# eladhoffer/convNet.pytorch

Hardware: NVIDIA H100
Metric: ResNet-50 images/sec (training step, synthetic 224x224) (higher is better)
Workload: dtype bf16

## Files before the change

### convnet/pytorch_b200/csrc/conv3x3.cu

```cuda
#include "common.cuh"
#include "host.h"
#include <stdlib.h>

namespace b200 {

constexpr int kHMaxA = 6, kHMaxB = 8;
constexpr int kHMaxTaps = 16;

struct HaloParams {
  int N, H, W, C, Kout;
  int RT, Wp;
  int tiles_per_img, m_tiles, n_tiles, block_n, c_chunks;
  int sa, sb;
  uint32_t a_bytes, a_box_bytes, b_bytes;
  int act;
  int has_res;
  double* stats;
  const float* bias;
  int ntaps, pad;
  int row_bytes;
  int b_stationary;
  int diag;
  uint16_t a_off[kHMaxTaps];
  uint16_t b_tap[kHMaxTaps];
};

template <int NTAPS, int KSTEPS, int BN>
__global__ void __launch_bounds__(kThreads, 1)
conv_halo_kernel(const __grid_constant__ CUtensorMap tmX, const __grid_constant__ CUtensorMap tmB,
                 const __grid_constant__ CUtensorMap tmC, const __grid_constant__ CUtensorMap tmR,
                 const __grid_constant__ HaloParams p) {
  extern __shared__ uint8_t smem_raw[];
  __shared__ __align__(8) uint64_t a_full[kHMaxA], a_empty[kHMaxA], b_full[kHMaxB], b_empty[kHMaxB];
  __shared__ __align__(8) uint64_t res_bar, bstat_bar;

  const int warp = threadIdx.x >> 5, lane = threadIdx.x & 31;
  const uint32_t raw_addr = smem_u32(smem_raw);
  uint8_t* smem = smem_raw + (((raw_addr + 1023u) & ~1023u) - raw_addr);
  uint8_t* sA = smem;
  uint8_t* sB = sA + p.sa * p.a_bytes;
  const int b_slots = p.b_stationary ? p.c_chunks * p.ntaps : p.sb;
  uint8_t* epi = sB + b_slots * p.b_bytes;

  if (threadIdx.x == 0) {
    for (int i = 0; i < p.sa; ++i) { mbar_init(&a_full[i], 1); mbar_init(&a_empty[i], 8); }
    for (int i = 0; i < kHMaxB; ++i) { mbar_init(&b_full[i], 1); mbar_init(&b_empty[i], 8); }
    mbar_init(&bstat_bar, 1);
    mbar_init(&res_bar, 1);
    fence_mbar_init();
    prefetch_tmap(&tmX); prefetch_tmap(&tmB); prefetch_tmap(&tmC);
    if (p.has_res) prefetch_tmap(&tmR);
  }
  __syncthreads();
  const int t_start = p.diag ? static_cast<int>(blockIdx.x) / p.n_tiles : static_cast<int>(blockIdx.x);
  const int t_step = p.diag ? static_cast<int>(gridDim.x) / p.n_tiles : static_cast<int>(gridDim.x);
  const int total_tiles = p.diag ? p.m_tiles : p.m_tiles * p.n_tiles;
  const int own_n = static_cast<int>(blockIdx.x) % p.n_tiles;

  if (warp >= 8) {
    producer_setmaxnreg();
    if (warp == 8 && lane == 0) {
      int ia = 0, ib = 0; uint32_t pa = 0, pb = 0;
      const int cw = p.row_bytes >> 1;
      if (p.b_stationary && t_start < total_tiles) {
        mbar_arrive_expect_tx(&bstat_bar, static_cast<uint32_t>(p.c_chunks * NTAPS) * p.b_bytes);
        for (int cc = 0; cc < p.c_chunks; ++cc)
          for (int t = 0; t < NTAPS; ++t)
            tma_load_3d(&tmB, &bstat_bar, sB + (cc * NTAPS + t) * p.b_bytes, cc * cw, p.b_tap[t],
                        p.diag ? own_n * p.block_n : 0);
      }
      for (int tile = t_start; tile < total_tiles; tile += t_step) {
        const int m_tile = p.diag ? tile : tile / p.n_tiles, n_tile = p.diag ? own_n : tile - m_tile * p.n_tiles;
        const int img = m_tile / p.tiles_per_img;
        const int h0 = (m_tile - img * p.tiles_per_img) * p.RT;
        for (int cc = 0; cc < p.c_chunks; ++cc) {
          mbar_wait(&a_empty[ia], pa ^ 1u);
          mbar_arrive_expect_tx(&a_full[ia], p.a_box_bytes);
          tma_load_4d(&tmX, &a_full[ia], sA + ia * p.a_bytes, (p.diag ? n_tile : cc) * cw, -p.pad, h0 - p.pad, img);
          if (++ia == p.sa) { ia = 0; pa ^= 1u; }
          if (p.b_stationary) continue;
          for (int t = 0; t < NTAPS; ++t) {
            mbar_wait(&b_empty[ib], pb ^ 1u);
            mbar_arrive_expect_tx(&b_full[ib], p.b_bytes);
            tma_load_3d(&tmB, &b_full[ib], sB + ib * p.b_bytes, cc * cw, p.b_tap[t], n_tile * p.block_n);
            if (++ib == p.sb) { ib = 0; pb ^= 1u; }
          }
        }
      }
    }
    return;
  }
  consumer_setmaxnreg();

  const int wg = warp >> 2;
  const int r_lo = wg * 64 + (warp & 3) * 16 + (lane >> 2);
  const int c_lo = 2 * (lane & 3);
  const bool leader = threadIdx.x == 0;
  const uint64_t proto = make_smem_desc(0, 16, 8u * p.row_bytes, layout_type_for_row_bytes(p.row_bytes));
  const uint32_t a_wg = (64u * wg * p.row_bytes) >> 4;
  const int nbox = BN >> 6;
  const uint32_t box_bytes = static_cast<uint32_t>(p.RT * p.W) * 128u;
  const uint32_t box_pitch = (box_bytes + 1023u) & ~1023u;
  int srow[2];
  bool in_tile[2];
#pragma unroll
  for (int h = 0; h < 2; ++h) {
    const int v = r_lo + 8 * h;
    const int ry = v / p.Wp, cx = v - ry * p.Wp;
    srow[h] = ry * p.W + cx;
    in_tile[h] = (ry < p.RT) && (cx < p.W);
  }
  const int st_col = threadIdx.x % BN;
  const int st_rows = kTileM / (256 / BN);
  const int st_row0 = (threadIdx.x / BN) * st_rows;
  int st_ntile = -1;
  float st_s1 = 0.f, st_s2 = 0.f;
  if (p.b_stationary && t_start < total_tiles) mbar_wait(&bstat_bar, 0);

  float acc[BN / 2];
  int ia = 0, ib = 0; uint32_t pa = 0, pb = 0;
  int local = 0;
  for (int tile = t_start; tile < total_tiles; tile += t_step, ++local) {
    const int m_tile = p.diag ? tile : tile / p.n_tiles, n_tile = p.diag ? own_n : tile - m_tile * p.n_tiles;
    const int img = m_tile / p.tiles_per_img;
    const int h0 = (m_tile - img * p.tiles_per_img) * p.RT;
    const int nbase = n_tile * BN;
    if (leader && local > 0) bulk_wait_group_read0();
    named_bar_sync(1, 256);
    if (leader && p.has_res) {
      fence_proxy_async();
      mbar_arrive_expect_tx(&res_bar, static_cast<uint32_t>(nbox) * box_bytes);
      for (int b = 0; b < nbox; ++b) tma_load_4d(&tmR, &res_bar, epi + b * box_pitch, nbase + b * 64, 0, h0, img);
    }

    wgmma_fence_acc(acc);
    int rel_a = -1, rel_b = -1;
    for (int cc = 0; cc < p.c_chunks; ++cc) {
      mbar_wait(&a_full[ia], pa);
      const uint64_t da0 = proto + (smem_u32(sA + ia * p.a_bytes) >> 4) + a_wg;
#pragma unroll
      for (int t = 0; t < NTAPS; ++t) {
        uint64_t db0;
        if (p.b_stationary) {
          db0 = proto + (smem_u32(sB + (cc * NTAPS + t) * p.b_bytes) >> 4);
        } else {
          mbar_wait(&b_full[ib], pb);
          db0 = proto + (smem_u32(sB + ib * p.b_bytes) >> 4);
        }
        const uint32_t tap_inc = (static_cast<uint32_t>(p.a_off[t]) * p.row_bytes) >> 4;
        wgmma_fence();
#pragma unroll
        for (int k = 0; k < KSTEPS; ++k)
          wgmma_bf16<0, 0>(acc, da0 + tap_inc + 2 * k, db0 + 2 * k, (cc | t | k) != 0 ? 1u : 0u);
        if (!p.b_stationary || t == NTAPS - 1) {
          wgmma_commit();
          wgmma_wait<1>();
          if (rel_b >= 0) release_stage(&b_empty[rel_b], lane);
          if (rel_a >= 0) release_stage(&a_empty[rel_a], lane);
          rel_a = (t == NTAPS - 1) ? ia : -1;
          rel_b = p.b_stationary ? -1 : ib;
        }
        if (!p.b_stationary && ++ib == p.sb) { ib = 0; pb ^= 1u; }
      }
      if (++ia == p.sa) { ia = 0; pa ^= 1u; }
    }
    wgmma_wait<0>();
    wgmma_fence_acc(acc);
    if (rel_b >= 0) release_stage(&b_empty[rel_b], lane);
    if (rel_a >= 0) release_stage(&a_empty[rel_a], lane);

    if (p.has_res) mbar_wait(&res_bar, static_cast<uint32_t>(local & 1));
#pragma unroll
    for (int h = 0; h < 2; ++h) {
      if (!in_tile[h] || h0 + (r_lo + 8 * h) / p.Wp >= p.H) continue;
      const int row = srow[h];
#pragma unroll
      for (int j = 0; j < BN / 2; j += 4) {
        const int c = 2 * j + c_lo;
        uint32_t* dst = reinterpret_cast<uint32_t*>(epi + staged_offset(row, c, box_pitch));
        float v0 = acc[j + 2 * h], v1 = acc[j + 2 * h + 1];
        if (p.bias != nullptr) { v0 += __ldg(p.bias + nbase + c); v1 += __ldg(p.bias + nbase + c + 1); }
        if (p.has_res) {
          const float2 t2 = unpack_bf16x2(*dst);
          v0 += t2.x;
          v1 += t2.y;
        }
        *dst = pack_bf16x2(apply_act(v0, p.act), apply_act(v1, p.act));
      }
    }
    fence_proxy_async();
    named_bar_sync(1, 256);
    if (leader) {
      for (int b = 0; b < nbox; ++b) tma_store_4d(&tmC, epi + b * box_pitch, nbase + b * 64, 0, h0, img);
      bulk_commit_group();
    }
    if (p.stats != nullptr) {
      if (st_ntile != n_tile) {
        if (st_ntile >= 0) flush_bn_stats(p.stats, p.Kout, st_ntile * BN, st_col, st_s1, st_s2);
        st_ntile = n_tile; st_s1 = 0.f; st_s2 = 0.f;
      }
      const int vrows = min(p.RT, p.H - h0) * p.W;
      const int r_end = min(st_row0 + st_rows, vrows);
      for (int r = st_row0; r < r_end; ++r) {
        const float x = __bfloat162float(*reinterpret_cast<const __nv_bfloat16*>(epi + staged_offset(r, st_col, box_pitch)));
        st_s1 += x;
        st_s2 = fmaf(x, x, st_s2);
      }
    }
  }
  if (p.stats != nullptr && st_ntile >= 0) flush_bn_stats(p.stats, p.Kout, st_ntile * BN, st_col, st_s1, st_s2);
  if (leader) bulk_wait_group0();
}

typedef void (*HaloKernelFn)(const __grid_constant__ CUtensorMap, const __grid_constant__ CUtensorMap,
                             const __grid_constant__ CUtensorMap, const __grid_constant__ CUtensorMap,
                             const __grid_constant__ HaloParams);
static HaloKernelFn halo_kernel_for(int ntaps, int block_n) {
  if (ntaps == 9)
    return block_n == 64 ? conv_halo_kernel<9, 4, 64> : block_n == 128 ? conv_halo_kernel<9, 4, 128>
         : block_n == 256 ? conv_halo_kernel<9, 4, 256> : nullptr;
  if (ntaps == 16)
    return block_n == 64 ? conv_halo_kernel<16, 1, 64> : block_n == 128 ? conv_halo_kernel<16, 1, 128>
         : block_n == 256 ? conv_halo_kernel<16, 1, 256> : nullptr;
  return nullptr;
}

bool halo_geometry_ok(int H, int W, int Cs, int R, int S, int pad) {
  const bool k3 = (R == 3 && S == 3 && pad == 1 && Cs % 64 == 0);
  const bool k4 = (R == 4 && S == 4 && pad == 0 && Cs == 16);
  if (!k3 && !k4) return false;
  const int Wp = W + S - 1;
  if (Wp > 128 || W < 8) return false;
  int RT = 128 / Wp;
  if (RT > H) RT = H;
  const int tiles = (H + RT - 1) / RT;
  return (double)H * W / (128.0 * tiles) >= 0.6;
}

bool halo_eligible(int H, int W, int Cs, int Nout, int R, int S, int pad) {
  if (!halo_geometry_ok(H, W, Cs, R, S, pad) || Nout % 64 != 0) return false;
  const int n_tiles = (Nout + 255) / 256;
  const int block_n = Nout / n_tiles;
  return Nout % n_tiles == 0 && block_n % 64 == 0 && 256 % block_n == 0;
}

int launch_halo(const void* src, const void* wmat, void* out, const void* res, const float* bias, int N, int H, int W,
                int Cs, int Nout, int R, int S, int pad, int dir, int act, double* stats, cudaStream_t stream, int window) {
  HaloParams p;
  memset(&p, 0, sizeof(p));
  p.diag = window > 0 ? 1 : 0;
  if (p.diag)
    B200_REQUIRE(window == 64 && Cs == Nout && Cs % 64 == 0 && R == 3 && S == 3, B200_ERR_UNSUPPORTED,
                 "conv halo: window mode needs window == 64, C == K, C %% 64 == 0 and a 3x3 filter (C=%d K=%d)", Cs, Nout);
  p.N = N; p.H = H; p.W = W; p.C = Cs; p.Kout = Nout;
  p.ntaps = R * S; p.pad = pad;
  p.row_bytes = (Cs == 16) ? 32 : 128;
  const int cw = p.row_bytes / 2;
  p.Wp = W + S - 1;
  p.RT = 128 / p.Wp;
  if (p.RT > H) p.RT = H;
  p.tiles_per_img = (H + p.RT - 1) / p.RT;
  p.m_tiles = N * p.tiles_per_img;
  p.n_tiles = p.diag ? Nout / 64 : (Nout + 255) / 256;
  p.block_n = Nout / p.n_tiles;
  p.c_chunks = p.diag ? 1 : Cs / cw;
  p.a_box_bytes = (uint32_t)(p.RT + R - 1) * p.Wp * p.row_bytes;
  uint32_t a_need = (uint32_t)(kTileM + (R - 1) * p.Wp + (S - 1)) * p.row_bytes;
  if (a_need < p.a_box_bytes) a_need = p.a_box_bytes;
  p.a_bytes = (a_need + 1023u) & ~1023u;
  p.b_bytes = (uint32_t)p.block_n * p.row_bytes;
  p.act = act;
  p.has_res = res != nullptr;
  p.stats = stats;
  p.bias = bias;
  for (int r = 0; r < R; ++r)
    for (int s = 0; s < S; ++s) {
      const int t = r * S + s;
      p.b_tap[t] = (uint16_t)t;
      p.a_off[t] = (uint16_t)(dir == 0 ? r * p.Wp + s : (R - 1 - r) * p.Wp + (S - 1 - s));
    }
  const uint32_t box_pitch = (((uint32_t)(p.RT * W) * 128u) + 1023u) & ~1023u;
  const uint32_t epi_bytes = (uint32_t)(p.block_n / 64) * box_pitch;
  int budget = 212 * 1024 - (int)epi_bytes;
  const int b_all = p.c_chunks * p.ntaps * (int)p.b_bytes;
  p.b_stationary = ((p.n_tiles == 1 || p.diag) && b_all <= 80 * 1024) ? 1 : 0;
  B200_REQUIRE(!p.diag || p.b_stationary, B200_ERR_UNSUPPORTED, "conv halo: window mode expects resident weights");
  int b_region;
  if (p.b_stationary) {
    b_region = b_all;
    p.sb = 0;
    p.sa = (budget - b_region) / (int)p.a_bytes;
    if (p.sa > kHMaxA) p.sa = kHMaxA;
  } else {
    p.sa = 2;
    p.sb = (budget - p.sa * (int)p.a_bytes) / (int)p.b_bytes;
    if (p.sb > kHMaxB) p.sb = kHMaxB;
    if (p.sb >= 6 && (int)(3 * p.a_bytes + 4 * p.b_bytes) <= budget) {
      p.sa = 3;
      p.sb = (budget - 3 * (int)p.a_bytes) / (int)p.b_bytes;
      if (p.sb > kHMaxB) p.sb = kHMaxB;
    }
    b_region = p.sb * (int)p.b_bytes;
  }
  B200_REQUIRE(p.sa >= 2 && (p.b_stationary || p.sb >= 2), B200_ERR_UNSUPPORTED,
               "conv halo: shared memory budget exceeded (W=%d, block_n=%d)", W, p.block_n);
  CUtensorMap tmX, tmB, tmC, tmR;
  memset(&tmR, 0, sizeof(tmR));
  int rc = encode_tiled(&tmX, src, 4, {Cs, W + S - 1 - 2 * pad, H + R - 1 - 2 * pad, N}, {cw, p.Wp, p.RT + R - 1, 1},
                        "conv halo source");
  if (rc) return rc;
  rc = encode_tiled(&tmB, wmat, 3, {p.diag ? window : Cs, p.ntaps, Nout}, {cw, 1, p.block_n}, "conv halo weights");
  if (rc) return rc;
  rc = encode_tiled(&tmC, out, 4, {Nout, W, H, N}, {64, W, p.RT, 1}, "conv halo output");
  if (rc) return rc;
  if (res) {
    rc = encode_tiled(&tmR, res, 4, {Nout, W, H, N}, {64, W, p.RT, 1}, "conv halo residual");
    if (rc) return rc;
  }
  const int smem_bytes = p.sa * (int)p.a_bytes + b_region + (int)epi_bytes + 1024;
  HaloKernelFn kfn = halo_kernel_for(p.ntaps, p.block_n);
  B200_REQUIRE(kfn != nullptr, B200_ERR_UNSUPPORTED, "conv halo: %d taps with block_n %d unsupported", p.ntaps, p.block_n);
  rc = set_smem_attr((const void*)kfn, smem_bytes);
  if (rc) return rc;
  const int total = p.m_tiles * p.n_tiles;
  int grid = total < sm_count() ? total : sm_count();
  if (p.diag) {
    int per_n = sm_count() / p.n_tiles;
    if (per_n > p.m_tiles) per_n = p.m_tiles;
    if (per_n < 1) per_n = 1;
    grid = per_n * p.n_tiles;
  }
  if (getenv("B200_HALO_DEBUG"))
    fprintf(stderr, "[halo] dir=%d N=%d H=%d W=%d C=%d K=%d taps=%d block_n=%d n_tiles=%d m_tiles=%d bstat=%d diag=%d "
            "sa=%d sb=%d bias=%d res=%d act=%d stats=%d grid=%d\n", dir, N, H, W, Cs, Nout, p.ntaps, p.block_n,
            p.n_tiles, p.m_tiles, p.b_stationary, p.diag, p.sa, p.sb, bias != nullptr, res != nullptr, act,
            stats != nullptr, grid);
  b200::launch(kfn, grid, kThreads, smem_bytes, stream, tmX, tmB, tmC, tmR, p);
  B200_CHECK_LAUNCH("conv_halo_kernel");
  return B200_OK;
}


constexpr int kWMaxStages = 4;

struct HaloWgradParams {
  int N, H, W, K_out, C;
  int RT, Wp, tiles_per_img, m_tiles;
  int ntaps, pad, halo_rows;
  int x_row_bytes, cw, ncols;
  int c_chunks, k_tiles, units, splits, tiles_per_split;
  int stages;
  int window;
  uint32_t a_box_bytes, a_bytes, x_box_bytes, x_bytes;
  float* partial;
  uint16_t x_off[kHMaxTaps];
};

template <int R, int S>
__global__ void __launch_bounds__(kThreads, 1)
conv_halo_wgrad_kernel(const __grid_constant__ CUtensorMap tmDy, const __grid_constant__ CUtensorMap tmX,
                       const __grid_constant__ HaloWgradParams p) {
  constexpr int kCols = S * 16;
  extern __shared__ uint8_t smem_raw[];
  __shared__ __align__(8) uint64_t full_bar[kWMaxStages], empty_bar[kWMaxStages];
  const int warp = threadIdx.x >> 5, lane = threadIdx.x & 31;
  const uint32_t raw_addr = smem_u32(smem_raw);
  uint8_t* smem = smem_raw + (((raw_addr + 1023u) & ~1023u) - raw_addr);
  const uint32_t stage_bytes = p.a_bytes + p.x_bytes;

  {
    uint4* z = reinterpret_cast<uint4*>(smem);
    const int n16 = static_cast<int>(p.stages * stage_bytes) >> 4;
    for (int i = threadIdx.x; i < n16; i += kThreads) z[i] = make_uint4(0u, 0u, 0u, 0u);
  }
  if (threadIdx.x == 0) {
    for (int s = 0; s < p.stages; ++s) { mbar_init(&full_bar[s], 1); mbar_init(&empty_bar[s], 8); }
    fence_mbar_init();
    prefetch_tmap(&tmDy);
    prefetch_tmap(&tmX);
  }
  fence_proxy_async();
  __syncthreads();

  const int split = blockIdx.x / p.units;
  const int unit = blockIdx.x - split * p.units;
  const int k_tile = unit % p.k_tiles;
  const int cc = unit / p.k_tiles;
  const int k0 = k_tile * kTileM;
  const int t_begin = split * p.tiles_per_split;
  const int t_end = min(p.m_tiles, t_begin + p.tiles_per_split);
  const int ntiles = t_end - t_begin;
  const int nA = min(2, (p.K_out - k0 + 63) / 64);
  if (ntiles <= 0) return;

  if (warp >= 8) {
    producer_setmaxnreg();
    if (warp == 8 && lane == 0) {
      int stage = 0; uint32_t phase = 0;
      const uint32_t tx = nA * p.a_box_bytes + p.x_box_bytes;
      for (int tile = t_begin; tile < t_end; ++tile) {
        const int img = tile / p.tiles_per_img;
        const int h0 = (tile - img * p.tiles_per_img) * p.RT;
        mbar_wait(&empty_bar[stage], phase ^ 1u);
        uint8_t* sa = smem + stage * stage_bytes;
        mbar_arrive_expect_tx(&full_bar[stage], tx);
        for (int j = 0; j < nA; ++j) tma_load_4d(&tmDy, &full_bar[stage], sa + j * 16384, k0 + j * 64, 0, h0, img);
        tma_load_4d(&tmX, &full_bar[stage], sa + p.a_bytes, cc * p.cw + (p.window ? k0 : 0), -p.pad, h0 - p.pad, img);
        if (++stage == p.stages) { stage = 0; phase ^= 1u; }
      }
    }
    return;
  }
  consumer_setmaxnreg();

  const int wg = warp >> 2;
  const bool wg_on = wg < nA;
  const uint64_t protoA = make_smem_desc(0, 16384, 1024, 1);
  const uint64_t protoX = make_smem_desc(0, p.x_row_bytes, 8u * p.x_row_bytes, layout_type_for_row_bytes(p.x_row_bytes));
  uint32_t row_inc[R];
#pragma unroll
  for (int r = 0; r < R; ++r) row_inc[r] = (static_cast<uint32_t>(p.x_off[r * S]) * p.x_row_bytes) >> 4;
  const uint32_t kx_inc = (16u * p.x_row_bytes) >> 4;
  float acc[R][kCols / 2];
#pragma unroll
  for (int r = 0; r < R; ++r) wgmma_fence_acc(acc[r]);
  int stage = 0, prev = 0; uint32_t phase = 0;
  for (int i = 0; i < ntiles; ++i) {
    mbar_wait(&full_bar[stage], phase);
    if (wg_on) {
      const uint32_t a_addr = smem_u32(smem + stage * stage_bytes);
      const uint64_t da0 = protoA + ((a_addr + wg * 16384) >> 4);
      const uint64_t dx0 = protoX + ((a_addr + p.a_bytes) >> 4);
      wgmma_fence();
#pragma unroll
      for (int k = 0; k < 8; ++k) {
        const uint32_t scale = (k != 0 || i != 0) ? 1u : 0u;
#pragma unroll
        for (int r = 0; r < R; ++r)
          wgmma_bf16<1, 1>(acc[r], da0 + k * 128, dx0 + row_inc[r] + k * kx_inc, scale);
      }
      wgmma_commit();
      wgmma_wait<1>();
    }
    if (i > 0) release_stage(&empty_bar[prev], lane);
    prev = stage;
    if (++stage == p.stages) { stage = 0; phase ^= 1u; }
  }
  wgmma_wait<0>();
#pragma unroll
  for (int r = 0; r < R; ++r) wgmma_fence_acc(acc[r]);
  release_stage(&empty_bar[prev], lane);
  if (!wg_on) return;

  const int row = wg * 64 + (warp & 3) * 16 + (lane >> 2);
  const int c_lo = 2 * (lane & 3);
#pragma unroll
  for (int h = 0; h < 2; ++h) {
    float* dst = p.partial + ((static_cast<long long>(unit) * p.splits + split) * kTileM + row + 8 * h) * p.ncols;
#pragma unroll
    for (int r = 0; r < R; ++r)
#pragma unroll
      for (int j = 0; j < kCols / 2; j += 4)
        *reinterpret_cast<float2*>(dst + r * kCols + 2 * j + c_lo) = make_float2(acc[r][j + 2 * h], acc[r][j + 2 * h + 1]);
  }
}

bool halo_wgrad_eligible(int H, int W, int C, int K_out, int R, int S, int pad, int window) {
  if (!halo_geometry_ok(H, W, C, R, S, pad) || K_out % 64 != 0) return false;
  const int units = ((window ? window : C) / 16) * ((K_out + kTileM - 1) / kTileM);
  return units <= sm_count() + 8;
}

int launch_halo_wgrad(const void* x, const void* dy, float* dw, void* workspace, size_t workspace_bytes, int N, int H,
                      int W, int C, int K_out, int R, int S, int pad, cudaStream_t stream, int window) {
  HaloWgradParams p;
  memset(&p, 0, sizeof(p));
  p.window = window;
  if (window)
    B200_REQUIRE(window == 128 && C == K_out && C % 128 == 0, B200_ERR_UNSUPPORTED,
                 "conv halo wgrad: window mode needs window == 128 and C == K, C %% 128 == 0 (C=%d K=%d)", C, K_out);
  p.N = N; p.H = H; p.W = W; p.K_out = K_out; p.C = C;
  p.ntaps = R * S; p.pad = pad;
  p.cw = 16;
  p.x_row_bytes = p.cw * 2;
  p.ncols = p.ntaps * p.cw;
  p.Wp = W + S - 1;
  p.RT = 128 / p.Wp;
  if (p.RT > H) p.RT = H;
  p.halo_rows = p.RT + R - 1;
  p.tiles_per_img = (H + p.RT - 1) / p.RT;
  p.m_tiles = N * p.tiles_per_img;
  p.c_chunks = (window ? window : C) / p.cw;
  p.k_tiles = (K_out + kTileM - 1) / kTileM;
  p.units = p.c_chunks * p.k_tiles;
  int splits = sm_count() / p.units;
  if (splits < 1) splits = 1;
  if (splits > p.m_tiles) splits = p.m_tiles;
  p.tiles_per_split = (p.m_tiles + splits - 1) / splits;
  p.splits = (p.m_tiles + p.tiles_per_split - 1) / p.tiles_per_split;
  p.a_box_bytes = (uint32_t)(p.RT * p.Wp) * 128u;
  p.a_bytes = 2 * 16384;
  p.x_box_bytes = (uint32_t)(p.halo_rows * p.Wp) * p.x_row_bytes;
  int max_off = 0;
  for (int r = 0; r < R; ++r)
    for (int s = 0; s < S; ++s) {
      p.x_off[r * S + s] = (uint16_t)(r * p.Wp + s);
      if (r * p.Wp + s > max_off) max_off = r * p.Wp + s;
    }
  uint32_t x_need = (uint32_t)(kTileM + max_off) * p.x_row_bytes;
  if (x_need < p.x_box_bytes) x_need = p.x_box_bytes;
  p.x_bytes = (x_need + 1023u) & ~1023u;
  p.stages = (212 * 1024) / (int)(p.a_bytes + p.x_bytes);
  if (p.stages > kWMaxStages) p.stages = kWMaxStages;
  B200_REQUIRE(p.stages >= 2, B200_ERR_UNSUPPORTED, "conv halo wgrad: shared memory budget exceeded (W=%d)", W);
  const size_t need = (size_t)p.units * p.splits * kTileM * p.ncols * sizeof(float);
  B200_REQUIRE(workspace != nullptr && workspace_bytes >= need, B200_ERR_INVALID,
               "conv halo wgrad: workspace of %zu bytes needed (%zu given)", need, workspace_bytes);
  p.partial = reinterpret_cast<float*>(workspace);
  CUtensorMap tmDy, tmX;
  int rc = encode_tiled(&tmDy, dy, 4, {K_out, W, H, N}, {64, p.Wp, p.RT, 1}, "conv halo wgrad dy");
  if (rc) return rc;
  rc = encode_tiled(&tmX, x, 4, {C, W + S - 1 - 2 * pad, H + R - 1 - 2 * pad, N}, {p.cw, p.Wp, p.halo_rows, 1},
                    "conv halo wgrad x");
  if (rc) return rc;
  const int smem_bytes = p.stages * (int)(p.a_bytes + p.x_bytes) + 1024;
  const auto kfn = p.ntaps == 9 ? conv_halo_wgrad_kernel<3, 3> : conv_halo_wgrad_kernel<4, 4>;
  rc = set_smem_attr((const void*)kfn, smem_bytes);
  if (rc) return rc;
  if (getenv("B200_HALO_DEBUG"))
    fprintf(stderr, "[halo_wgrad] N=%d H=%d W=%d C=%d K=%d taps=%d k_tiles=%d c_chunks=%d m_tiles=%d units=%d "
            "splits=%d tiles_per_split=%d stages=%d grid=%d window=%d\n", N, H, W, C, K_out, p.ntaps, p.k_tiles,
            p.c_chunks, p.m_tiles, p.units, p.splits, p.tiles_per_split, p.stages, p.units * p.splits, window);
  b200::launch(kfn, p.units * p.splits, kThreads, smem_bytes, stream, tmDy, tmX, p);
  B200_CHECK_LAUNCH("conv_halo_wgrad_kernel");
  return launch_wgrad_reduce(p.partial, dw, K_out, p.ntaps, window ? window : C, p.cw, 1, p.ntaps, p.ntaps, p.k_tiles,
                             p.splits, p.ncols, stream);
}

}
```

Measured before the change: 6579.

## Widen halo wgrad channel chunks and keep both warpgroups busy on half K tiles

For 3x3 weight gradients, each CTA now processes 32 input channels per chunk instead of 16, which doubles the wgmma N width and halves the number of units. When K_out leaves a 64-row tail tile, the second warpgroup is no longer idle. It either takes half of the filter rows (even R) or a second channel chunk loaded into an extra X slot (odd R). The split count is also capped by the available workspace. Together these aim to raise tensor-core utilization and cut idle warpgroups, at the cost of more accumulator registers per thread and larger shared-memory stages, which may reduce pipeline depth.

```diff
diff --git a/convnet/pytorch_b200/csrc/conv3x3.cu b/convnet/pytorch_b200/csrc/conv3x3.cu
--- a/convnet/pytorch_b200/csrc/conv3x3.cu
+++ b/convnet/pytorch_b200/csrc/conv3x3.cu
@@ -347,30 +347,43 @@
   int N, H, W, K_out, C;
   int RT, Wp, tiles_per_img, m_tiles;
   int ntaps, pad, halo_rows;
-  int x_row_bytes, cw, ncols;
+  int x_row_bytes, ncols;
   int c_chunks, k_tiles, units, splits, tiles_per_split;
+  int half;
+  int works;
   int stages;
   int window;
-  uint32_t a_box_bytes, a_bytes, x_box_bytes, x_bytes;
+  uint32_t a_box_bytes, a_bytes, x_box_bytes, x_bytes, stage_bytes;
   float* partial;
   uint16_t x_off[kHMaxTaps];
 };
 
-template <int R, int S>
+template <int NR, int R, int NC>
+__device__ __forceinline__ void halo_wgrad_mmas(float (&acc)[R][NC], uint64_t da0, uint64_t dx0,
+                                                const uint32_t (&row_inc)[R], uint32_t kx_inc, bool accumulate) {
+#pragma unroll
+  for (int k = 0; k < 8; ++k) {
+    const uint32_t scale = (k != 0 || accumulate) ? 1u : 0u;
+#pragma unroll
+    for (int r = 0; r < NR; ++r) wgmma_bf16<1, 1>(acc[r], da0 + k * 128, dx0 + row_inc[r] + k * kx_inc, scale);
+  }
+}
+
+template <int R, int S, int CW>
 __global__ void __launch_bounds__(kThreads, 1)
 conv_halo_wgrad_kernel(const __grid_constant__ CUtensorMap tmDy, const __grid_constant__ CUtensorMap tmX,
                        const __grid_constant__ HaloWgradParams p) {
-  constexpr int kCols = S * 16;
+  constexpr int kCols = S * CW;
+  constexpr bool kRowSplit = (R % 2 == 0);
   extern __shared__ uint8_t smem_raw[];
   __shared__ __align__(8) uint64_t full_bar[kWMaxStages], empty_bar[kWMaxStages];
   const int warp = threadIdx.x >> 5, lane = threadIdx.x & 31;
   const uint32_t raw_addr = smem_u32(smem_raw);
   uint8_t* smem = smem_raw + (((raw_addr + 1023u) & ~1023u) - raw_addr);
-  const uint32_t stage_bytes = p.a_bytes + p.x_bytes;
 
   {
     uint4* z = reinterpret_cast<uint4*>(smem);
-    const int n16 = static_cast<int>(p.stages * stage_bytes) >> 4;
+    const int n16 = static_cast<int>(p.stages * p.stage_bytes) >> 4;
     for (int i = threadIdx.x; i < n16; i += kThreads) z[i] = make_uint4(0u, 0u, 0u, 0u);
   }
   if (threadIdx.x == 0) {
@@ -382,30 +395,35 @@
   fence_proxy_async();
   __syncthreads();
 
-  const int split = blockIdx.x / p.units;
-  const int unit = blockIdx.x - split * p.units;
-  const int k_tile = unit % p.k_tiles;
-  const int cc = unit / p.k_tiles;
+  const int split = blockIdx.x / p.works;
+  const int work = blockIdx.x - split * p.works;
+  const int kt_full = p.k_tiles - p.half;
+  const bool half = work >= kt_full * p.c_chunks;
+  const int k_tile = half ? kt_full : work % kt_full;
+  const int cc = half ? (work - kt_full * p.c_chunks) * (kRowSplit ? 1 : 2) : work / kt_full;
+  const bool pair = half && !kRowSplit;
   const int k0 = k_tile * kTileM;
   const int t_begin = split * p.tiles_per_split;
   const int t_end = min(p.m_tiles, t_begin + p.tiles_per_split);
   const int ntiles = t_end - t_begin;
-  const int nA = min(2, (p.K_out - k0 + 63) / 64);
   if (ntiles <= 0) return;
 
   if (warp >= 8) {
     producer_setmaxnreg();
     if (warp == 8 && lane == 0) {
       int stage = 0; uint32_t phase = 0;
-      const uint32_t tx = nA * p.a_box_bytes + p.x_box_bytes;
+      const int nA = half ? 1 : 2, nX = pair ? 2 : 1;
+      const uint32_t tx = nA * p.a_box_bytes + nX * p.x_box_bytes;
       for (int tile = t_begin; tile < t_end; ++tile) {
         const int img = tile / p.tiles_per_img;
         const int h0 = (tile - img * p.tiles_per_img) * p.RT;
         mbar_wait(&empty_bar[stage], phase ^ 1u);
-        uint8_t* sa = smem + stage * stage_bytes;
+        uint8_t* sa = smem + stage * p.stage_bytes;
         mbar_arrive_expect_tx(&full_bar[stage], tx);
         for (int j = 0; j < nA; ++j) tma_load_4d(&tmDy, &full_bar[stage], sa + j * 16384, k0 + j * 64, 0, h0, img);
-        tma_load_4d(&tmX, &full_bar[stage], sa + p.a_bytes, cc * p.cw + (p.window ? k0 : 0), -p.pad, h0 - p.pad, img);
+        for (int j = 0; j < nX; ++j)
+          tma_load_4d(&tmX, &full_bar[stage], sa + p.a_bytes + j * p.x_bytes, (cc + j) * CW + (p.window ? k0 : 0),
+                      -p.pad, h0 - p.pad, img);
         if (++stage == p.stages) { stage = 0; phase ^= 1u; }
       }
     }
@@ -414,12 +432,17 @@
   consumer_setmaxnreg();
 
   const int wg = warp >> 2;
-  const bool wg_on = wg < nA;
+  const uint32_t a_off = half ? 0u : static_cast<uint32_t>(wg) * 16384u;
+  const uint32_t x_slot = pair ? static_cast<uint32_t>(wg) * p.x_bytes : 0u;
+  const bool split_rows = kRowSplit && half;
+  const int r0 = split_rows ? wg * (R / 2) : 0;
+  const int nr = split_rows ? R / 2 : R;
   const uint64_t protoA = make_smem_desc(0, 16384, 1024, 1);
   const uint64_t protoX = make_smem_desc(0, p.x_row_bytes, 8u * p.x_row_bytes, layout_type_for_row_bytes(p.x_row_bytes));
   uint32_t row_inc[R];
 #pragma unroll
-  for (int r = 0; r < R; ++r) row_inc[r] = (static_cast<uint32_t>(p.x_off[r * S]) * p.x_row_bytes) >> 4;
+  for (int r = 0; r < R; ++r)
+    row_inc[r] = (static_cast<uint32_t>(p.x_off[min(r0 + r, R - 1) * S]) * p.x_row_bytes) >> 4;
   const uint32_t kx_inc = (16u * p.x_row_bytes) >> 4;
   float acc[R][kCols / 2];
 #pragma unroll
@@ -427,21 +450,14 @@
   int stage = 0, prev = 0; uint32_t phase = 0;
   for (int i = 0; i < ntiles; ++i) {
     mbar_wait(&full_bar[stage], phase);
-    if (wg_on) {
-      const uint32_t a_addr = smem_u32(smem + stage * stage_bytes);
-      const uint64_t da0 = protoA + ((a_addr + wg * 16384) >> 4);
-      const uint64_t dx0 = protoX + ((a_addr + p.a_bytes) >> 4);
-      wgmma_fence();
-#pragma unroll
-      for (int k = 0; k < 8; ++k) {
-        const uint32_t scale = (k != 0 || i != 0) ? 1u : 0u;
-#pragma unroll
-        for (int r = 0; r < R; ++r)
-          wgmma_bf16<1, 1>(acc[r], da0 + k * 128, dx0 + row_inc[r] + k * kx_inc, scale);
-      }
-      wgmma_commit();
-      wgmma_wait<1>();
-    }
+    const uint32_t a_addr = smem_u32(smem + stage * p.stage_bytes);
+    const uint64_t da0 = protoA + ((a_addr + a_off) >> 4);
+    const uint64_t dx0 = protoX + ((a_addr + p.a_bytes + x_slot) >> 4);
+    wgmma_fence();
+    if (split_rows) halo_wgrad_mmas<R / 2>(acc, da0, dx0, row_inc, kx_inc, i != 0);
+    else halo_wgrad_mmas<R>(acc, da0, dx0, row_inc, kx_inc, i != 0);
+    wgmma_commit();
+    wgmma_wait<1>();
     if (i > 0) release_stage(&empty_bar[prev], lane);
     prev = stage;
     if (++stage == p.stages) { stage = 0; phase ^= 1u; }
@@ -450,24 +466,28 @@
 #pragma unroll
   for (int r = 0; r < R; ++r) wgmma_fence_acc(acc[r]);
   release_stage(&empty_bar[prev], lane);
-  if (!wg_on) return;
-
-  const int row = wg * 64 + (warp & 3) * 16 + (lane >> 2);
+
+  const int unit = (cc + (pair ? wg : 0)) * p.k_tiles + k_tile;
+  const int row = (half ? 0 : wg * 64) + (warp & 3) * 16 + (lane >> 2);
   const int c_lo = 2 * (lane & 3);
 #pragma unroll
   for (int h = 0; h < 2; ++h) {
     float* dst = p.partial + ((static_cast<long long>(unit) * p.splits + split) * kTileM + row + 8 * h) * p.ncols;
 #pragma unroll
     for (int r = 0; r < R; ++r)
-#pragma unroll
-      for (int j = 0; j < kCols / 2; j += 4)
-        *reinterpret_cast<float2*>(dst + r * kCols + 2 * j + c_lo) = make_float2(acc[r][j + 2 * h], acc[r][j + 2 * h + 1]);
-  }
-}
+      if (r < nr)
+#pragma unroll
+        for (int j = 0; j < kCols / 2; j += 4)
+          *reinterpret_cast<float2*>(dst + (r0 + r) * kCols + 2 * j + c_lo) =
+              make_float2(acc[r][j + 2 * h], acc[r][j + 2 * h + 1]);
+  }
+}
+
+static int halo_wgrad_cw(int R) { return R == 4 ? 16 : 32; }
 
 bool halo_wgrad_eligible(int H, int W, int C, int K_out, int R, int S, int pad, int window) {
   if (!halo_geometry_ok(H, W, C, R, S, pad) || K_out % 64 != 0) return false;
-  const int units = ((window ? window : C) / 16) * ((K_out + kTileM - 1) / kTileM);
+  const int units = ((window ? window : C) / halo_wgrad_cw(R)) * ((K_out + kTileM - 1) / kTileM);
   return units <= sm_count() + 8;
 }
 
@@ -479,27 +499,36 @@
   if (window)
     B200_REQUIRE(window == 128 && C == K_out && C % 128 == 0, B200_ERR_UNSUPPORTED,
                  "conv halo wgrad: window mode needs window == 128 and C == K, C %% 128 == 0 (C=%d K=%d)", C, K_out);
+  B200_REQUIRE(K_out % 64 == 0, B200_ERR_UNSUPPORTED, "conv halo wgrad: K=%d must be a multiple of 64", K_out);
   p.N = N; p.H = H; p.W = W; p.K_out = K_out; p.C = C;
   p.ntaps = R * S; p.pad = pad;
-  p.cw = 16;
-  p.x_row_bytes = p.cw * 2;
-  p.ncols = p.ntaps * p.cw;
+  const int cw = halo_wgrad_cw(R);
+  p.x_row_bytes = cw * 2;
+  p.ncols = p.ntaps * cw;
   p.Wp = W + S - 1;
   p.RT = 128 / p.Wp;
   if (p.RT > H) p.RT = H;
   p.halo_rows = p.RT + R - 1;
   p.tiles_per_img = (H + p.RT - 1) / p.RT;
   p.m_tiles = N * p.tiles_per_img;
-  p.c_chunks = (window ? window : C) / p.cw;
+  p.c_chunks = (window ? window : C) / cw;
   p.k_tiles = (K_out + kTileM - 1) / kTileM;
   p.units = p.c_chunks * p.k_tiles;
-  int splits = sm_count() / p.units;
+  p.half = (K_out % kTileM == 64) ? 1 : 0;
+  const bool row_split = (R % 2 == 0);
+  B200_REQUIRE(!p.half || row_split || p.c_chunks % 2 == 0, B200_ERR_UNSUPPORTED,
+               "conv halo wgrad: an odd chunk count (%d) cannot pair", p.c_chunks);
+  p.works = (p.k_tiles - p.half) * p.c_chunks + (p.half ? (row_split ? p.c_chunks : p.c_chunks / 2) : 0);
+  const size_t slot = (size_t)kTileM * p.ncols * sizeof(float);
+  int splits = sm_count() / p.works;
+  const int ws_splits = (int)(workspace_bytes / (slot * p.units));
+  if (splits > ws_splits) splits = ws_splits;
   if (splits < 1) splits = 1;
   if (splits > p.m_tiles) splits = p.m_tiles;
   p.tiles_per_split = (p.m_tiles + splits - 1) / splits;
   p.splits = (p.m_tiles + p.tiles_per_split - 1) / p.tiles_per_split;
   p.a_box_bytes = (uint32_t)(p.RT * p.Wp) * 128u;
-  p.a_bytes = 2 * 16384;
+  p.a_bytes = K_out > 64 ? 2 * 16384 : 16384;
   p.x_box_bytes = (uint32_t)(p.halo_rows * p.Wp) * p.x_row_bytes;
   int max_off = 0;
   for (int r = 0; r < R; ++r)
@@ -510,30 +539,34 @@
   uint32_t x_need = (uint32_t)(kTileM + max_off) * p.x_row_bytes;
   if (x_need < p.x_box_bytes) x_need = p.x_box_bytes;
   p.x_bytes = (x_need + 1023u) & ~1023u;
-  p.stages = (212 * 1024) / (int)(p.a_bytes + p.x_bytes);
+  const int pair = (p.half && !row_split) ? 1 : 0;
+  p.stage_bytes = p.a_bytes + (1 + pair) * p.x_bytes;
+  p.stages = (212 * 1024) / (int)p.stage_bytes;
   if (p.stages > kWMaxStages) p.stages = kWMaxStages;
   B200_REQUIRE(p.stages >= 2, B200_ERR_UNSUPPORTED, "conv halo wgrad: shared memory budget exceeded (W=%d)", W);
-  const size_t need = (size_t)p.units * p.splits * kTileM * p.ncols * sizeof(float);
+  const size_t need = (size_t)p.units * p.splits * slot;
   B200_REQUIRE(workspace != nullptr && workspace_bytes >= need, B200_ERR_INVALID,
                "conv halo wgrad: workspace of %zu bytes needed (%zu given)", need, workspace_bytes);
   p.partial = reinterpret_cast<float*>(workspace);
   CUtensorMap tmDy, tmX;
   int rc = encode_tiled(&tmDy, dy, 4, {K_out, W, H, N}, {64, p.Wp, p.RT, 1}, "conv halo wgrad dy");
   if (rc) return rc;
-  rc = encode_tiled(&tmX, x, 4, {C, W + S - 1 - 2 * pad, H + R - 1 - 2 * pad, N}, {p.cw, p.Wp, p.halo_rows, 1},
+  rc = encode_tiled(&tmX, x, 4, {C, W + S - 1 - 2 * pad, H + R - 1 - 2 * pad, N}, {cw, p.Wp, p.halo_rows, 1},
                     "conv halo wgrad x");
   if (rc) return rc;
-  const int smem_bytes = p.stages * (int)(p.a_bytes + p.x_bytes) + 1024;
-  const auto kfn = p.ntaps == 9 ? conv_halo_wgrad_kernel<3, 3> : conv_halo_wgrad_kernel<4, 4>;
+  const int smem_bytes = p.stages * (int)p.stage_bytes + 1024;
+  const auto kfn = p.ntaps == 9 ? conv_halo_wgrad_kernel<3, 3, 32> : conv_halo_wgrad_kernel<4, 4, 16>;
   rc = set_smem_attr((const void*)kfn, smem_bytes);
   if (rc) return rc;
+  const int grid = p.works * p.splits;
   if (getenv("B200_HALO_DEBUG"))
     fprintf(stderr, "[halo_wgrad] N=%d H=%d W=%d C=%d K=%d taps=%d k_tiles=%d c_chunks=%d m_tiles=%d units=%d "
-            "splits=%d tiles_per_split=%d stages=%d grid=%d window=%d\n", N, H, W, C, K_out, p.ntaps, p.k_tiles,
-            p.c_chunks, p.m_tiles, p.units, p.splits, p.tiles_per_split, p.stages, p.units * p.splits, window);
-  b200::launch(kfn, p.units * p.splits, kThreads, smem_bytes, stream, tmDy, tmX, p);
+            "splits=%d tiles_per_split=%d stages=%d grid=%d window=%d cw=%d pair=%d row_split=%d works=%d\n", N, H, W,
+            C, K_out, p.ntaps, p.k_tiles, p.c_chunks, p.m_tiles, p.units, p.splits, p.tiles_per_split, p.stages, grid,
+            window, cw, pair, (p.half && row_split) ? 1 : 0, p.works);
+  b200::launch(kfn, grid, kThreads, smem_bytes, stream, tmDy, tmX, p);
   B200_CHECK_LAUNCH("conv_halo_wgrad_kernel");
-  return launch_wgrad_reduce(p.partial, dw, K_out, p.ntaps, window ? window : C, p.cw, 1, p.ntaps, p.ntaps, p.k_tiles,
+  return launch_wgrad_reduce(p.partial, dw, K_out, p.ntaps, window ? window : C, cw, 1, p.ntaps, p.ntaps, p.k_tiles,
                              p.splits, p.ncols, stream);
 }
 
```

After: 6601, median of 6. No clear change (+0.3%).
